# CompVis/zigma

Measured on AMD Instinct MI355X. Metric: denoiser-forward latents/sec (BxL tokens/s), ZigMa d=640 L=32^2, higher is better.
Workload: dtype bf16; 1 GPU; readme_text_b64: ZigMa(in_ch=3,img=32,E=640,depth=18,zigzagN8,has_text 77x768), B=64/GPU, bf16, one forward per step; global_batch=64, seq_len=1024, parallelism=batch-sharded x1

## Files before the change

include/zigma_hip.h:

```cpp
#ifndef ZIGMA_HIP_H_
#define ZIGMA_HIP_H_

#include <stdint.h>

#ifdef __cplusplus
extern "C" {
#endif

#define ZIGMA_ABI_VERSION 10

#define ZIGMA_SCAN_Z_PREACTIVATED 2
#define ZIGMA_SCAN_ACCUMULATE 4
#define ZIGMA_SCAN_PROBE_V1 0x100
#define ZIGMA_SCAN_PROBE_PRIO_SHIFT 9
#define ZIGMA_SCAN_PROBE_R5_SHIFT 10

#define ZIGMA_SCAN_KERNEL_GENERIC 1
#define ZIGMA_SCAN_KERNEL_TOK 2
#define ZIGMA_SCAN_KERNEL_TOK2 3

typedef enum zigma_status {
    ZIGMA_OK = 0,
    ZIGMA_ERR_NULL = -1,
    ZIGMA_ERR_SHAPE = -2,
// ... 202 lines not shown

int zigma_scale_reduce_bwd(const zigma_glue_bwd_params_t *p, void *stream);

typedef struct zigma_xattn_params {
    int32_t batch, seqlen, n_ctx, heads, head_dim;
    int32_t dtype;
    int32_t flags;
    float scale;
    int64_t q_batch_stride, q_row_stride;
    int64_t k_batch_stride, k_row_stride;
    int64_t v_batch_stride, v_row_stride;
    int64_t o_batch_stride, o_row_stride;
    const void *q, *k, *v;
    void *out;
} zigma_xattn_params_t;

int zigma_cross_attn_fwd(const zigma_xattn_params_t *p, void *stream);

typedef struct zigma_xattn_bwd_params {
    int32_t batch, seqlen, n_ctx, heads, head_dim;
    int32_t dtype;
    int32_t flags;
    float scale;
    int32_t chunks;
    int32_t pad_;
    int64_t q_batch_stride, q_row_stride;
    int64_t k_batch_stride, k_row_stride;
    int64_t v_batch_stride, v_row_stride;
    int64_t do_batch_stride, do_row_stride;
    int64_t dq_batch_stride, dq_row_stride;
    const void *q, *k, *v, *dout;
    void *dq, *dk_part, *dv_part;
} zigma_xattn_bwd_params_t;

int zigma_cross_attn_bwd_chunks(int seqlen);
int zigma_cross_attn_bwd(const zigma_xattn_bwd_params_t *p, void *stream);

typedef struct zigma_xproj_params {
    int64_t m;
    int32_t n, k;
    int32_t dtype;
    int32_t flags;
    int64_t x_row_stride, w_row_stride, out_row_stride;
    const void *x, *w;
    void *out;
} zigma_xproj_params_t;

int zigma_x_proj_fwd(const zigma_xproj_params_t *p, void *stream);

typedef struct zigma_conv_xproj_params {
    int32_t batch, seqlen, dim, n;
    int32_t dtype;
    int32_t flags;
    int64_t x_batch_stride, x_l_stride;
    int64_t u_batch_stride, u_l_stride;
    int64_t w_row_stride, out_row_stride;
    const void *x, *conv_weight, *conv_bias, *w;
    void *u, *out;
    const int32_t *x_row_index;
} zigma_conv_xproj_params_t;

int zigma_conv_x_proj_fwd(const zigma_conv_xproj_params_t *p, void *stream);

#define ZIGMA_LINEAR_WS 0x4000
#define ZIGMA_LINEAR_SM 0x8000
typedef struct zigma_linear_params {
    int64_t m;
    int32_t n, k;
    int32_t dtype;
    int32_t flags;
    int32_t silu_from_col;
    int32_t pad_;
    int64_t x_row_stride, w_row_stride, out_row_stride;
    const void *x, *w;
    const void *bias;
    void *out;
    const void *residual, *gate;
    int64_t res_row_stride, gate_batch_stride;
    int32_t rows_per_batch, pad2_;
} zigma_linear_params_t;

int zigma_linear_fwd(const zigma_linear_params_t *p, void *stream);

typedef struct zigma_linear_wgrad_params {
    int64_t m;
    int32_t n, k;
    int32_t dtype;
    int32_t out_dtype;
    int32_t slabs;
    int32_t flags;
    int64_t dy_row_stride, x_row_stride, out_row_stride;
    const void *dy, *x;
    void *out;
    void *workspace;
    int64_t workspace_bytes;
} zigma_linear_wgrad_params_t;

int64_t zigma_linear_wgrad_workspace_bytes(const zigma_linear_wgrad_params_t *p);
int zigma_linear_wgrad(const zigma_linear_wgrad_params_t *p, void *stream);

typedef struct zigma_linear_split_params {
    int64_t m;
    int32_t n, k;
    int32_t passes;
    int32_t flags;
    int64_t x_row_stride, w_hi_row_stride, w_lo_row_stride, out_row_stride;
    const void *x;
    const void *w_hi, *w_lo;
    const void *bias;
    void *out;
} zigma_linear_split_params_t;

int zigma_linear_f32_split(const zigma_linear_split_params_t *p, void *stream);

typedef struct zigma_patch_embed_params {
    int32_t batch, in_chans, height, width, patch, embed_dim;
    int32_t dtype;
    int32_t flags;
    int64_t x_batch_stride, x_chan_stride, x_row_stride;
    int64_t pos_row_stride, out_batch_stride, out_row_stride;
    const void *x, *weight, *bias, *pos;
    void *out;
} zigma_patch_embed_params_t;

typedef struct zigma_timestep_embed_params {
    int32_t batch, dim;
    int32_t dtype;
    int32_t flags;
    int64_t out_row_stride;
    const void *t, *freqs;
    void *out;
} zigma_timestep_embed_params_t;

typedef struct zigma_final_layer_params {
    int64_t rows;
    int32_t cols, n_out;
    int32_t dtype;
    int32_t flags;
    float eps;
    int32_t pad_;
    int64_t x_row_stride, out_row_stride;
    const void *x, *weight, *bias;
    void *out;
} zigma_final_layer_params_t;

typedef struct zigma_skinny_params {
    int32_t m, n, k;
    int32_t dtype;
    int32_t flags;
    int32_t pad_;
    int64_t x_row_stride, w_row_stride, out_row_stride;
    const void *x, *w, *bias;
    void *out;
} zigma_skinny_params_t;

int zigma_patch_embed_fwd(const zigma_patch_embed_params_t *p, void *stream);
int zigma_timestep_embed_fwd(const zigma_timestep_embed_params_t *p, void *stream);
int zigma_final_layer_fwd(const zigma_final_layer_params_t *p, void *stream);
int zigma_skinny_linear_fwd(const zigma_skinny_params_t *p, void *stream);

typedef struct zigma_calib_params {
    int32_t mode, iters;
    int64_t bytes;
    const void *src;
    void *dst;
} zigma_calib_params_t;
// ... 11 lines not shown
```

zigma_amd/_lib.py:

```python
import ctypes as C
import os

import torch

_HERE = os.path.dirname(os.path.abspath(__file__))
LIB_PATH = os.environ.get("ZIGMA_AMD_LIB") or os.path.join(_HERE, "lib", "libzigma_hip.so")

F32, F16, BF16 = 0, 1, 2
_DT = {torch.float32: F32, torch.float16: F16, torch.bfloat16: BF16}

i32, i64, vp, f32 = C.c_int32, C.c_int64, C.c_void_p, C.c_float


class ScanParams(C.Structure):
    _fields_ = (
        [(n, i32) for n in ("batch", "dim", "seqlen", "dstate", "n_groups", "is_variable_B", "is_variable_C",
                            "delta_softplus", "io_dtype", "bc_dtype", "chunk_len", "flags")]
        + [(n, i64) for n in (
            "u_batch_stride", "u_d_stride", "u_l_stride",
            "delta_batch_stride", "delta_d_stride", "delta_l_stride",
            "z_batch_stride", "z_d_stride", "z_l_stride",
            "out_batch_stride", "out_d_stride", "out_l_stride",
            "out_z_batch_stride", "out_z_d_stride", "out_z_l_stride",
            "A_d_stride", "A_dstate_stride",
# ... 65 lines not shown
    _fields_ = ([(n, i32) for n in ("rows", "cols", "is_rms", "x_dtype", "res_dtype", "w_dtype")]
                + [("eps", f32), ("flags", i32)]
                + [(n, i64) for n in ("xsum_row_stride", "dy_row_stride", "dres_out_row_stride", "dx_row_stride",
                                      "dres_row_stride")]
                + [(n, vp) for n in ("xsum", "weight", "dy", "dresidual_out", "dx", "dresidual", "dweight", "dbias",
                                     "workspace")]
                + [("workspace_bytes", i64)])


class XAttnParams(C.Structure):
    _fields_ = ([(n, i32) for n in ("batch", "seqlen", "n_ctx", "heads", "head_dim", "dtype", "flags")] + [("scale", f32)]
                + [(n, i64) for n in ("q_batch_stride", "q_row_stride", "k_batch_stride", "k_row_stride", "v_batch_stride",
                                      "v_row_stride", "o_batch_stride", "o_row_stride")]
                + [(n, vp) for n in ("q", "k", "v", "out")])


class XAttnBwdParams(C.Structure):
    _fields_ = ([(n, i32) for n in ("batch", "seqlen", "n_ctx", "heads", "head_dim", "dtype", "flags")] + [("scale", f32)]
                + [("chunks", i32), ("pad_", i32)]
                + [(n, i64) for n in ("q_batch_stride", "q_row_stride", "k_batch_stride", "k_row_stride", "v_batch_stride",
                                      "v_row_stride", "do_batch_stride", "do_row_stride", "dq_batch_stride", "dq_row_stride")]
                + [(n, vp) for n in ("q", "k", "v", "dout", "dq", "dk_part", "dv_part")])


class PatchEmbedParams(C.Structure):
    _fields_ = ([(n, i32) for n in ("batch", "in_chans", "height", "width", "patch", "embed_dim", "dtype", "flags")]
                + [(n, i64) for n in ("x_batch_stride", "x_chan_stride", "x_row_stride", "pos_row_stride", "out_batch_stride", "out_row_stride")]
                + [(n, vp) for n in ("x", "weight", "bias", "pos", "out")])


class TimestepEmbedParams(C.Structure):
    _fields_ = [("batch", i32), ("dim", i32), ("dtype", i32), ("flags", i32), ("out_row_stride", i64), ("t", vp), ("freqs", vp), ("out", vp)]


class FinalLayerParams(C.Structure):
    _fields_ = ([("rows", i64), ("cols", i32), ("n_out", i32), ("dtype", i32), ("flags", i32), ("eps", f32), ("pad_", i32),
                 ("x_row_stride", i64), ("out_row_stride", i64)] + [(n, vp) for n in ("x", "weight", "bias", "out")])


class SkinnyParams(C.Structure):
    _fields_ = ([(n, i32) for n in ("m", "n", "k", "dtype", "flags", "pad_")] + [(n, i64) for n in ("x_row_stride", "w_row_stride", "out_row_stride")]
                + [(n, vp) for n in ("x", "w", "bias", "out")])


class GlueBwdParams(C.Structure):
    _fields_ = ([("rows", i64), ("cols", i32), ("rows_per_batch", i32), ("dtype", i32), ("flags", i32), ("s_add", f32), ("pad_", i32)]
                + [(n, i64) for n in ("dy_row_stride", "a_row_stride", "out_row_stride", "s_batch_stride")]
                + [(n, vp) for n in ("dy", "a", "s", "out", "r1", "r2")])


class CalibParams(C.Structure):
    _fields_ = [("mode", i32), ("iters", i32), ("bytes", i64), ("src", vp), ("dst", vp)]


class XProjParams(C.Structure):
    _fields_ = ([("m", i64), ("n", i32), ("k", i32), ("dtype", i32), ("flags", i32)]
                + [(n, i64) for n in ("x_row_stride", "w_row_stride", "out_row_stride")] + [(n, vp) for n in ("x", "w", "out")])


class ConvXProjParams(C.Structure):
    _fields_ = ([(n, i32) for n in ("batch", "seqlen", "dim", "n", "dtype", "flags")]
                + [(n, i64) for n in ("x_batch_stride", "x_l_stride", "u_batch_stride", "u_l_stride", "w_row_stride", "out_row_stride")]
                + [(n, vp) for n in ("x", "conv_weight", "conv_bias", "w", "u", "out", "x_row_index")])


class LinearParams(C.Structure):
    _fields_ = ([("m", i64), ("n", i32), ("k", i32), ("dtype", i32), ("flags", i32), ("silu_from_col", i32), ("pad_", i32)]
                + [(n, i64) for n in ("x_row_stride", "w_row_stride", "out_row_stride")] + [(n, vp) for n in ("x", "w", "bias", "out")]
                + [("residual", vp), ("gate", vp), ("res_row_stride", i64), ("gate_batch_stride", i64), ("rows_per_batch", i32), ("pad2_", i32)])


class LinearWgradParams(C.Structure):
    _fields_ = ([("m", i64), ("n", i32), ("k", i32), ("dtype", i32), ("out_dtype", i32), ("slabs", i32), ("flags", i32)]
                + [(n, i64) for n in ("dy_row_stride", "x_row_stride", "out_row_stride")] + [(n, vp) for n in ("dy", "x", "out", "workspace")]
                + [("workspace_bytes", i64)])


class LinearSplitParams(C.Structure):
    _fields_ = ([("m", i64), ("n", i32), ("k", i32), ("passes", i32), ("flags", i32)]
                + [(n, i64) for n in ("x_row_stride", "w_hi_row_stride", "w_lo_row_stride", "out_row_stride")]
                + [(n, vp) for n in ("x", "w_hi", "w_lo", "bias", "out")])


EXPORTS = ("zigma_linear_fwd", "zigma_linear_f32_split", "zigma_linear_wgrad","zigma_linear_wgrad_workspace_bytes", "zigma_conv_x_proj_fwd", "zigma_scale_reduce_bwd", "zigma_selective_scan_fwd", "zigma_causal_conv1d_fwd", "zigma_add_norm_fwd", "zigma_dt_proj_softplus_fwd", "zigma_cross_attn_fwd", "zigma_x_proj_fwd", "zigma_selective_scan_bwd",
           "zigma_selective_scan_bwd_workspace_bytes", "zigma_causal_conv1d_bwd",
           "zigma_causal_conv1d_bwd_workspace_bytes", "zigma_add_norm_bwd", "zigma_add_norm_bwd_workspace_bytes",
           "zigma_strerror",
           "zigma_cross_attn_bwd", "zigma_cross_attn_bwd_chunks", "zigma_patch_embed_fwd", "zigma_timestep_embed_fwd", "zigma_final_layer_fwd",
           "zigma_skinny_linear_fwd", "zigma_calib_launch", "zigma_abi_version", "zigma_last_kernel")

_lib = None


def lib():
    global _lib
    if _lib is None:
        if not os.path.exists(LIB_PATH):
            raise RuntimeError(
                f"zigma_amd: {LIB_PATH} not built — run `python -m zigma_amd.build` (hipcc, gfx950). "
                "There is no CPU or eager fallback for the HIP ops.")
        L = C.CDLL(LIB_PATH)
        for name, st in (("zigma_selective_scan_fwd", ScanParams), ("zigma_causal_conv1d_fwd", ConvParams),
                         ("zigma_add_norm_fwd", NormParams), ("zigma_dt_proj_softplus_fwd", DtProjParams),
                         ("zigma_selective_scan_bwd", ScanBwdParams), ("zigma_causal_conv1d_bwd", ConvBwdParams),
                         ("zigma_add_norm_bwd", NormBwdParams), ("zigma_cross_attn_fwd", XAttnParams), ("zigma_cross_attn_bwd", XAttnBwdParams), ("zigma_patch_embed_fwd", PatchEmbedParams),
                         ("zigma_timestep_embed_fwd", TimestepEmbedParams), ("zigma_final_layer_fwd", FinalLayerParams), ("zigma_skinny_linear_fwd", SkinnyParams), ("zigma_x_proj_fwd", XProjParams),
                         ("zigma_linear_fwd", LinearParams), ("zigma_conv_x_proj_fwd", ConvXProjParams), ("zigma_scale_reduce_bwd", GlueBwdParams), ("zigma_calib_launch", CalibParams),
                         ("zigma_linear_wgrad", LinearWgradParams), ("zigma_linear_f32_split", LinearSplitParams)):
            fn = getattr(L, name)
            fn.argtypes = [C.POINTER(st), vp]
            fn.restype = C.c_int
        for name, st in (("zigma_selective_scan_bwd_workspace_bytes", ScanBwdParams),
                         ("zigma_causal_conv1d_bwd_workspace_bytes", ConvBwdParams),
                         ("zigma_add_norm_bwd_workspace_bytes", NormBwdParams),
                         ("zigma_linear_wgrad_workspace_bytes", LinearWgradParams)):
            fn = getattr(L, name)
            fn.argtypes = [C.POINTER(st)]
            fn.restype = C.c_int64
        L.zigma_cross_attn_bwd_chunks.argtypes = [C.c_int]
        L.zigma_cross_attn_bwd_chunks.restype = C.c_int
        L.zigma_strerror.argtypes = [C.c_int]
        L.zigma_strerror.restype = C.c_char_p
        L.zigma_abi_version.restype = C.c_int
        L.zigma_last_kernel.restype = C.c_char_p
        if L.zigma_abi_version() != 10:
            raise RuntimeError("zigma_amd: libzigma_hip.so ABI version mismatch")
        _lib = L
    return _lib


def last_kernel():
    return lib().zigma_last_kernel().decode()


def dtype_id(t):
    try:
        return _DT[t.dtype]
    except KeyError:
        raise RuntimeError(f"zigma_amd: unsupported dtype {t.dtype}")


def ptr(t):
    return None if t is None else t.data_ptr()


def require_device(*tensors):
    dev = None
    for t in tensors:
        if t is None:
            continue
        if not t.is_cuda:
            raise RuntimeError("zigma_amd: HIP kernels need tensors on a GPU device (no CPU fallback); got a "
                               f"{t.device} tensor")
        if dev is None:
            dev = t.device
        elif t.device != dev:
            raise RuntimeError("zigma_amd: all tensors must be on the same device")
    return dev


def workspace(fn_name, params, device):
    nbytes = getattr(lib(), fn_name + "_workspace_bytes")(C.byref(params))
    ws = torch.empty(max(int(nbytes), 16), device=device, dtype=torch.uint8)
    params.workspace, params.workspace_bytes = ws.data_ptr(), nbytes
    return ws


TRACE = None


def call(fn_name, params, device):
    L = lib()
    with torch.cuda.device(device):
        stream = torch.cuda.current_stream(device).cuda_stream
        rc = getattr(L, fn_name)(C.byref(params), C.c_void_p(stream))
    if rc != 0:
        raise RuntimeError(f"{fn_name}: {L.zigma_strerror(rc).decode()} (status {rc})")
    if TRACE is not None:
        TRACE.append((fn_name, L.zigma_last_kernel().decode(), params))
```

zigma_amd/build.py:

```python
import hashlib
import os
import subprocess
import sys
from concurrent.futures import ThreadPoolExecutor

HERE = os.path.dirname(os.path.abspath(__file__))
ROOT = os.path.dirname(HERE)
CSRC = os.path.join(HERE, "csrc")
OBJ = os.path.join(HERE, "build")
LIB = os.path.join(HERE, "lib", "libzigma_hip.so")
SOURCES = ["api.hip", "selective_scan.hip", "scan_tok_bf16.hip", "scan_tok_f16.hip", "scan_tok_f32.hip",
           "causal_conv1d.hip", "add_norm.hip", "dt_proj.hip", "scan_bwd.hip", "conv_bwd.hip", "norm_bwd.hip", "cross_attn.hip", "cross_attn_bwd.hip", "x_proj.hip", "linear.hip", "linear4w.hip", "linear_ws.hip", "linear_sm.hip", "conv_x_proj.hip", "glue_bwd.hip", "embed.hip", "skinny_linear.hip", "calib.hip", "wgrad.hip", "linear_split.hip"]
HIPCC = os.environ.get("HIPCC", "/opt/rocm/bin/hipcc")
FLAGS = ["--offload-arch=gfx950", "-O3", "-std=c++17", "-fPIC", "-ffp-contract=fast", "-fno-slp-vectorize",
         "-I" + os.path.join(ROOT, "include"), "-I" + CSRC]


_VGPR_MFMA = ["-mllvm", "-amdgpu-mfma-vgpr-form=1"]
_RES = ["-Rpass-analysis=kernel-resource-usage"]
SOURCE_FLAGS = {"cross_attn.hip": _VGPR_MFMA, "scan_tok_bf16.hip": _RES, "scan_tok_f16.hip": _RES, "wgrad.hip": _RES, "linear_split.hip": _RES}
NO_SCRATCH_KERNELS = ("scan_tok2_kernel", "wgrad_kernel", "wgrad_reduce_kernel", "linear_split_kernel")


def check_no_scratch(remarks, src):
    import re
    bad, seen, name = [], 0, None
    for ln in remarks.splitlines():
        m = re.search(r"remark: Function Name: (\S+)", ln)
        if m:
            name = m.group(1) if any(k in m.group(1) for k in NO_SCRATCH_KERNELS) else None
            seen += name is not None
            continue
        m = re.search(r"remark:\s+(ScratchSize \[bytes/lane\]|SGPRs Spill|VGPRs Spill): (\d+)", ln)
        if m and name and int(m.group(2)) != 0:
            bad.append((name, m.group(1), int(m.group(2))))
    if bad or not seen:
        raise RuntimeError(f"{src}: {' / '.join(NO_SCRATCH_KERNELS)} must not spill or use scratch (scan_tok2_kernel: inline-asm d16_hi row loads are invisible to the register allocator): "
                           f"{bad if bad else 'no instantiation found in the remarks'}")
    return seen


GENERATED_F16_INC = os.path.join(CSRC, "linear4w_body_f16.inc")


def ensure_generated(verbose=True):
    import importlib.util
    spec = importlib.util.spec_from_file_location("zigma_linear4w_gen", os.path.join(CSRC, "gen", "linear4w_gen.py"))
    gen = importlib.util.module_from_spec(spec)
    spec.loader.exec_module(gen)
    tmp = GENERATED_F16_INC + ".tmp"
    gen.emit_inc_f16(tmp)
    if os.path.exists(GENERATED_F16_INC) and open(GENERATED_F16_INC).read() == open(tmp).read():
        os.remove(tmp)
        return GENERATED_F16_INC
    os.replace(tmp, GENERATED_F16_INC)
    if verbose:
        print(f"generated {GENERATED_F16_INC}", flush=True)
    return GENERATED_F16_INC


def _digest(paths, extra=()):
    h = hashlib.sha256()
    for pth in sorted(paths):
        h.update(os.path.basename(pth).encode())
        h.update(open(pth, "rb").read())
    for e in extra:
        h.update(str(e).encode())
    return h.hexdigest()


def build(force=False, verbose=True, sources=None, lib=None, extra_flags=()):
    sources = sources or SOURCES
    lib = lib or LIB
    obj_dir = OBJ if lib == LIB else OBJ + "_" + os.path.splitext(os.path.basename(lib))[0]
    os.makedirs(obj_dir, exist_ok=True)
    os.makedirs(os.path.dirname(lib), exist_ok=True)
    ensure_generated(verbose)
    headers = [os.path.join(CSRC, f) for f in os.listdir(CSRC) if f.endswith((".h", ".inc"))]
    headers.append(os.path.join(ROOT, "include", "zigma_hip.h"))
    stamp = lib + ".srchash"
    want = _digest([os.path.join(CSRC, s) for s in sources] + headers, extra=list(FLAGS) + list(extra_flags) + [str(sorted(SOURCE_FLAGS.items()))])
    if not force and os.path.exists(lib) and os.path.exists(stamp) and open(stamp).read().strip() == want:
        if verbose:
            print(f"{lib} is up to date (source hash {want[:12]})")
        return lib

    def run(cmd):
        if verbose:
            print(" ".join(cmd), flush=True)
        subprocess.run(cmd, check=True)

    objs, jobs = [], []
    for src in sources:
        s_path = os.path.join(CSRC, src)
        o_path = os.path.join(obj_dir, src.replace(".hip", ".o"))
        o_stamp = o_path + ".srchash"
        src_flags = SOURCE_FLAGS.get(src, [])
        o_want = _digest([s_path] + headers, extra=list(FLAGS) + list(extra_flags) + src_flags)
        objs.append(o_path)
        if force or not os.path.exists(o_path) or not os.path.exists(o_stamp) or open(o_stamp).read().strip() != o_want:
            jobs.append(([HIPCC, *FLAGS, *extra_flags, *src_flags, "-c", s_path, "-o", o_path], o_stamp, o_want))

    def compile_one(job):
        cmd, o_stamp, o_want = job
# ... 21 lines not shown
```

zigma_amd/model_zigma.py:

```python
import math
import os
from functools import partial
from typing import Optional

import numpy as np
import torch
import torch.nn as nn
import torch.nn.functional as F
import torch.utils.checkpoint
from torch import Tensor

from .attention import attention_math, cross_attn, cross_attn_bwd_eligible, cross_attn_eligible, cross_attn_train
from . import embed as _embed
from .layernorm import RMSNorm, block_norm, glue_bwd_eligible, layer_norm_fn, rms_norm_fn, scale_reduce_bwd
from .linear import plan, project, run
from .mamba_simple import Mamba
from .scan_paths import hilbert_path, reverse_permut_np, zigzag_path


def modulate(x, shift, scale):
    return x * (1 + scale.unsqueeze(1)) + shift.unsqueeze(1)


class _ModulateFn(torch.autograd.Function):

    @staticmethod
    def forward(ctx, x, shift, scale):
        ctx.save_for_backward(x, scale)
        return torch.addcmul(shift.unsqueeze(1), x, (1 + scale).unsqueeze(1))

    @staticmethod
    def backward(ctx, dy):
        x, scale = ctx.saved_tensors
        if glue_bwd_eligible(dy, x, scale):
            dx, dscale, dshift = scale_reduce_bwd(dy, x, scale, s_add=1.0, want_sum=True)
            return dx, dshift, dscale
        dx = dy * (1 + scale).unsqueeze(1)
        return dx, dy.sum(1), (dy * x).sum(1)


class _GatedAddFn(torch.autograd.Function):

    @staticmethod
    def forward(ctx, base, gate, branch):
        ctx.save_for_backward(gate, branch)
        return torch.addcmul(base, gate.unsqueeze(1), branch)

    @staticmethod
    def backward(ctx, dy):
        gate, branch = ctx.saved_tensors
        if glue_bwd_eligible(dy, branch, gate):
            dbranch, dgate, _ = scale_reduce_bwd(dy, branch, gate)
            return dy, dgate, dbranch
        return dy, (dy * branch).sum(1), dy * gate.unsqueeze(1)


class PatchEmbed(nn.Module):

    def __init__(self, img_size=224, patch_size=16, in_chans=3, embed_dim=768, bias=True):
        super().__init__()
        self.img_size = (img_size, img_size)
        self.patch_size = (patch_size, patch_size)
        self.grid_size = (img_size // patch_size, img_size // patch_size)
        self.num_patches = self.grid_size[0] * self.grid_size[1]
        self.proj = nn.Conv2d(in_chans, embed_dim, kernel_size=patch_size, stride=patch_size, bias=bias)

    def forward(self, x, pos=None):
        Bsz, Cin, H, W = x.shape
        p = self.patch_size[0]
        no_grad = not (torch.is_grad_enabled() and (x.requires_grad or self.proj.weight.requires_grad
                                                    or (self.proj.bias is not None and self.proj.bias.requires_grad) or (pos is not None and pos.requires_grad)))
        if no_grad and _embed.patch_embed_eligible(x, self.proj.weight, self.proj.bias, pos):
            return _embed.patch_embed(x, self.proj.weight, self.proj.bias, pos)
        cols = x.reshape(Bsz, Cin, H // p, p, W // p, p).permute(0, 2, 4, 1, 3, 5).reshape(Bsz, -1, Cin * p * p)
        tok = F.linear(cols, self.proj.weight.reshape(self.proj.weight.shape[0], -1), self.proj.bias)
        return tok if pos is None else tok + pos


class PatchEmbed_Video(PatchEmbed):
    def forward(self, x, pos=None):
        Bsz, T = x.shape[:2]
        tok = super().forward(x.reshape((Bsz * T,) + x.shape[2:]))
        tok = tok.reshape(Bsz, -1, tok.shape[-1])
        return tok if pos is None else tok + pos


class CrossAttention(nn.Module):
    def __init__(self, query_dim, context_dim=None, heads=8, dim_head=64, dropout=0.0):
        super().__init__()
        inner_dim = dim_head * heads
        context_dim = query_dim if context_dim is None else context_dim
        self.scale = dim_head ** -0.5
        self.heads = heads
        self.to_q = nn.Linear(query_dim, inner_dim, bias=False)
        self.to_k = nn.Linear(context_dim, inner_dim, bias=False)
        self.to_v = nn.Linear(context_dim, inner_dim, bias=False)
        self.to_out = nn.Sequential(nn.Linear(inner_dim, query_dim), nn.Dropout(dropout))

    def _proj_out(self, o, residual, gate):
        lin = self.to_out[0]
        if residual is None or self.training:
            y = self.to_out[1](project("to_out", o, lin.weight, lin.bias))
            return y if residual is None else torch.addcmul(residual, gate.unsqueeze(1), y)
        return project("to_out", o, lin.weight, lin.bias, residual=residual, gate=gate)

    def forward(self, x, text, mask=None, kv=None, residual=None, gate=None):
        Bsz, L, _ = x.shape
        H = self.heads
        k, v = kv[:2] if kv is not None else (self.to_k(text), self.to_v(text))
        q = project("to_q", x, self.to_q.weight, self.to_q.bias)
        needs_grad = torch.is_grad_enabled() and (q.requires_grad or k.requires_grad or v.requires_grad)
        if cross_attn_eligible(q, k, v, H) and (not needs_grad or cross_attn_bwd_eligible(q, k, v, H)):
            if needs_grad:
                return self._proj_out(cross_attn_train(q, k, v, H, self.scale), residual, gate)
            return self._proj_out(cross_attn(q, k, v, H, self.scale), residual, gate)
        return self._proj_out(attention_math(q, k.reshape(Bsz, k.shape[1], -1), v.reshape(Bsz, v.shape[1], -1), H, self.scale), residual, gate)


def drop_path(x, drop_prob: float = 0.0, training: bool = False, scale_by_keep: bool = True):
    if drop_prob == 0.0 or not training:
        return x
    keep = 1 - drop_prob
    mask = x.new_empty((x.shape[0],) + (1,) * (x.ndim - 1)).bernoulli_(keep)
    if keep > 0.0 and scale_by_keep:
        mask.div_(keep)
    return x * mask


class DropPath(nn.Module):
    def __init__(self, drop_prob: float = 0.0, scale_by_keep: bool = True):
        super().__init__()
        self.drop_prob = drop_prob
        self.scale_by_keep = scale_by_keep

    def forward(self, x):
        return drop_path(x, self.drop_prob, self.training, self.scale_by_keep)


class TimestepEmbedder(nn.Module):

    def __init__(self, hidden_size, dtype, frequency_embedding_size=256):
        super().__init__()
        self.mlp = nn.Sequential(nn.Linear(frequency_embedding_size, hidden_size, bias=True), nn.SiLU(),
                                 nn.Linear(hidden_size, hidden_size, bias=True))
        self.dtype = dtype
        self.frequency_embedding_size = frequency_embedding_size
        self.register_buffer("_freqs", self.frequencies(frequency_embedding_size, dtype), persistent=False)

    @staticmethod
    def frequencies(dim, dtype, max_period=10000):
        half = dim // 2
        return torch.exp(-math.log(max_period) * torch.arange(start=0, end=half, dtype=dtype) / half)

    @staticmethod
    def timestep_embedding(t, dim, dtype, max_period=10000, freqs=None):
        if freqs is None:
            freqs = TimestepEmbedder.frequencies(dim, dtype, max_period).to(device=t.device)
        args = t[:, None].float() * freqs[None]
        embedding = torch.cat([torch.cos(args), torch.sin(args)], dim=-1)
        if dim % 2:
            embedding = torch.cat([embedding, torch.zeros_like(embedding[:, :1])], dim=-1)
        return embedding

    def forward(self, t):
        freqs = self._freqs if self._freqs.dtype == self.dtype else self._freqs.to(self.dtype)
        l1, l2 = self.mlp[0], self.mlp[2]
        if self.frequency_embedding_size % 2 == 0 and _embed.timestep_embed_eligible(t, freqs):
            t_freq = _embed.timestep_embed(t, freqs, self.frequency_embedding_size)
        else:
            t_freq = self.timestep_embedding(t, self.frequency_embedding_size, dtype=self.dtype, freqs=freqs).to(dtype=self.dtype)
        if _embed.skinny_linear_eligible(t_freq, l1.weight, l1.bias):
            h = _embed.skinny_linear(t_freq, l1.weight, l1.bias)
            if _embed.skinny_linear_eligible(h, l2.weight, l2.bias):
                return _embed.skinny_linear(h, l2.weight, l2.bias, silu=True)
            return l2(F.silu(h))
        return self.mlp(t_freq)


class LabelEmbedder(nn.Module):
    def __init__(self, num_classes, hidden_size, dropout_prob):
        super().__init__()
        use_cfg_embedding = dropout_prob > 0
        self.embedding_table = nn.Embedding(num_classes + use_cfg_embedding, hidden_size)
        self.num_classes = num_classes
        self.dropout_prob = dropout_prob

    def token_drop(self, labels, force_drop_ids=None):
        if force_drop_ids is None:
            drop_ids = torch.rand(labels.shape[0], device=labels.device) < self.dropout_prob
        else:
            drop_ids = force_drop_ids == 1
        return torch.where(drop_ids, self.num_classes, labels)

    def forward(self, labels, train, force_drop_ids=None):
        if (train and self.dropout_prob > 0) or (force_drop_ids is not None):
            labels = self.token_drop(labels, force_drop_ids)
        return self.embedding_table(labels)


class FinalLayer(nn.Module):
    def __init__(self, hidden_size, patch_size, out_channels, cond=False):
        super().__init__()
        self.norm_final = nn.LayerNorm(hidden_size, elementwise_affine=False, eps=1e-6)
        self.linear = nn.Linear(hidden_size, patch_size * patch_size * out_channels, bias=True)
        if cond:
            self.adaLN_modulation = nn.Sequential(nn.SiLU(), nn.Linear(hidden_size, 2 * hidden_size, bias=True))

    def forward(self, x, c=None):
        if c is None and _embed.final_layer_eligible(x, self.linear.weight, self.linear.bias):
            return _embed.final_layer(x, self.linear.weight, self.linear.bias, self.norm_final.eps)
        x = layer_norm_fn(x, None, None, eps=self.norm_final.eps)
        if c is not None:
            shift, scale = self.adaLN_modulation(c).chunk(2, dim=1)
            x = modulate(x, shift, scale)
        return self.linear(x)


class Pending:
    __slots__ = ("base", "branch", "gate")

    def __init__(self, base, branch=None, gate=None):
        self.base, self.branch, self.gate = base, branch, gate

    def materialize(self):
        if self.branch is None:
            return self.base
        return torch.addcmul(self.base, self.gate.unsqueeze(1), self.branch)


def _text_linear(x, weight, bias=None):
    k = x.shape[-1]
    m = x.numel() // k
    xp = x.new_zeros(-(-m // 256) * 256, k)
    xp[:m] = x.reshape(m, k)
    r = plan("text", xp, weight, bias)
    if r.kernel == "library":
        return F.linear(x, weight, bias)
    return run(r, xp, weight, bias)[:m].view(*x.shape[:-1], weight.shape[0])


FUSE_OUT_PROJ_ADD = True
FUSE_OUT_PROJ_ADD_NO_TEXT = True
from . import _knobs
_knobs.apply(globals(), "model_zigma")


class Block(nn.Module):
    def __init__(self, dim, mixer_cls, has_text=False, norm_cls=nn.LayerNorm, fused_add_norm=False,
                 residual_in_fp32=False, drop_path=0.0, skip=False):
        super().__init__()
        self.residual_in_fp32 = residual_in_fp32
        self.fused_add_norm = fused_add_norm
        self.has_text = has_text
        self.mixer = mixer_cls(dim)
        self.norm = norm_cls(dim)
        self.drop_path = DropPath(drop_path) if drop_path > 0.0 else nn.Identity()
        if self.fused_add_norm:
            assert isinstance(self.norm, (nn.LayerNorm, RMSNorm)), "Only LayerNorm and RMSNorm are supported for fused_add_norm"
        self.skip_linear = nn.Linear(2 * dim, dim) if skip else None
        adaln_num = 3 * 2 if self.has_text else 3
        self.adaLN_modulation = nn.Sequential(nn.SiLU(), nn.Linear(dim, adaln_num * dim, bias=True))
        if self.has_text:
            self.msa = CrossAttention(query_dim=dim, context_dim=dim, heads=8, dim_head=64, dropout=0.0)
            self.norm_msa = nn.LayerNorm(dim, elementwise_affine=False, eps=1e-6)

    def forward_fused(self, pend: Pending, residual, c, text=None, mod=None, kv=None):
        E = pend.base.shape[-1]
        if mod is None:
            mod = self.adaLN_modulation(c)
        is_rms = isinstance(self.norm, RMSNorm)
        _, residual, n, xm = block_norm(pend.base, self.norm.weight, self.norm.bias, residual, self.norm.eps, is_rms,
                                        residual_in_fp32=self.residual_in_fp32, branch=pend.branch, gate=pend.gate,
                                        shift=mod[:, 0:E], scale=mod[:, E:2 * E])
        g = mod[:, 2 * E:3 * E]
        fuse = FUSE_OUT_PROJ_ADD if self.has_text else FUSE_OUT_PROJ_ADD_NO_TEXT
        y, fused = self.mixer.forward_gated(xm, n, g) if fuse else (self.mixer(xm), False)
        pend = Pending(y) if fused else Pending(n, y, g)
        if not self.has_text:
            return pend, residual
        h, _, _, xa = block_norm(pend.base, None, None, None, self.norm_msa.eps, False, residual_in_fp32=False, branch=pend.branch,
                                 gate=pend.gate, shift=mod[:, 3 * E:4 * E], scale=mod[:, 4 * E:5 * E], want_x=True, want_y=False, want_res_out=False)
        h = pend.base if fused else h
        return Pending(self.msa(xa, text=text, mask=None, kv=kv, residual=h, gate=mod[:, 5 * E:6 * E])), residual

    def forward(self, x: Tensor, residual: Optional[Tensor] = None, c=None, text=None, inference_params=None, skip=None):
        if self.skip_linear is not None:
            x = self.skip_linear(torch.cat([x, skip], dim=-1))
        if not self.fused_add_norm:
            residual = x if residual is None else residual + self.drop_path(x)
            n = self.norm(residual.to(dtype=self.norm.weight.dtype))
            if self.residual_in_fp32:
                residual = residual.to(torch.float32)
            mod = self.adaLN_modulation(c).chunk(6 if self.has_text else 3, dim=1)
            h = n + mod[2].unsqueeze(1) * self.mixer(modulate(n, mod[0], mod[1]))
            if self.has_text:
                xa = modulate(layer_norm_fn(h, None, None, eps=self.norm_msa.eps), mod[3], mod[4])
                h = h + mod[5].unsqueeze(1) * self.msa(xa, text=text, mask=None)
            return h, residual
        if torch.is_grad_enabled() and (x.requires_grad or any(q.requires_grad for q in self.parameters())):
            return self.forward_train(x, residual, c, text)
        if residual is not None:
            x = self.drop_path(x)
        pend, residual = self.forward_fused(Pending(x), residual, c, text)
        return pend.materialize(), residual

    def forward_train(self, x, residual, c, text=None):
        fn = rms_norm_fn if isinstance(self.norm, RMSNorm) else layer_norm_fn
        x, residual = fn(x if residual is None else self.drop_path(x), self.norm.weight, self.norm.bias, residual=residual,
                         prenorm=True, residual_in_fp32=self.residual_in_fp32, eps=self.norm.eps)
        mod = self.adaLN_modulation(c).chunk(6 if self.has_text else 3, dim=1)
        x = _GatedAddFn.apply(x, mod[2], self.mixer(_ModulateFn.apply(x, mod[0], mod[1])))
        if self.has_text:
            xa = _ModulateFn.apply(layer_norm_fn(x, None, None, eps=self.norm_msa.eps), mod[3], mod[4])
            x = _GatedAddFn.apply(x, mod[5], self.msa(xa, text=text, mask=None))
        return x, residual


def create_block(d_model, ssm_cfg=None, has_text=False, norm_epsilon=1e-5, drop_path=0.0, rms_norm=False,
                 residual_in_fp32=False, fused_add_norm=False, skip=False, layer_idx=None, device=None, dtype=None,
                 scan_type="none", **block_kwargs):
    if ssm_cfg is None:
        ssm_cfg = {}
    factory_kwargs = {"device": device, "dtype": dtype}
    mixer_cls = partial(Mamba, layer_idx=layer_idx, scan_type=scan_type, **ssm_cfg, **block_kwargs, **factory_kwargs)
    norm_cls = partial(nn.LayerNorm if not rms_norm else RMSNorm, eps=norm_epsilon, **factory_kwargs)
    block = Block(d_model, mixer_cls, has_text=has_text, norm_cls=norm_cls, drop_path=drop_path,
                  fused_add_norm=fused_add_norm, residual_in_fp32=residual_in_fp32, skip=skip)
    block.layer_idx = layer_idx
    return block


def _init_weights(module, n_layer, initializer_range=0.02, rescale_prenorm_residual=True, n_residuals_per_layer=1):
    if isinstance(module, nn.Linear):
        if module.bias is not None and not getattr(module.bias, "_no_reinit", False):
            nn.init.zeros_(module.bias)
    elif isinstance(module, nn.Embedding):
        nn.init.normal_(module.weight, std=initializer_range)
    if rescale_prenorm_residual:
        for name, p in module.named_parameters():
            if name in ["out_proj.weight", "fc2.weight"]:
                nn.init.kaiming_uniform_(p, a=math.sqrt(5))
                with torch.no_grad():
                    p /= math.sqrt(n_residuals_per_layer * n_layer)


def get_1d_sincos_pos_embed_from_grid(embed_dim, pos):
    assert embed_dim % 2 == 0
    omega = 1.0 / 10000 ** (np.arange(embed_dim // 2, dtype=np.float64) / (embed_dim / 2.0))
    out = np.outer(pos.reshape(-1), omega)
    return np.concatenate([np.sin(out), np.cos(out)], axis=1)


def get_2d_sincos_pos_embed(embed_dim, grid_size, cls_token=False, extra_tokens=0):
    coords = np.arange(grid_size, dtype=np.float32)
    gw, gh = np.meshgrid(coords, coords)
    emb = np.concatenate([get_1d_sincos_pos_embed_from_grid(embed_dim // 2, gw),
                          get_1d_sincos_pos_embed_from_grid(embed_dim // 2, gh)], axis=1)
    if cls_token and extra_tokens > 0:
        emb = np.concatenate([np.zeros([extra_tokens, embed_dim]), emb], axis=0)
    return emb


# ... 235 lines not shown
```

Baseline: 3.772 million tokens/s.

## Fuse cross-attention LayerNorm and adaLN modulate into the to_q GEMM

Adds a new HIP kernel that computes LayerNorm and the shift/scale modulation on each 32-token tile, keeping the normalized rows in registers and feeding them straight into MFMA matmuls against the to_q weight (N=512). The goal is to stop materializing the modulated activation for cross-attention, saving a global write and read and a separate norm kernel launch per text block. It applies only in bias-free, no-grad, fused-pending cases above a token threshold, and falls back to the old path otherwise. The kernel is hand-scheduled (LDS staging, manual waitcnts) for fixed N and K, so it risks lower GEMM efficiency than the tuned library or routed kernel.

New measurement: 3.912 million tokens/s (median of 6 runs). +3.7%, better.

```diff
diff --git a/include/zigma_hip.h b/include/zigma_hip.h
--- a/include/zigma_hip.h
+++ b/include/zigma_hip.h
@@ -308,6 +308,20 @@
 
 int zigma_linear_fwd(const zigma_linear_params_t *p, void *stream);
 
+typedef struct zigma_norm_linear_params {
+    int64_t m;
+    int32_t n, k;
+    int32_t dtype;
+    int32_t flags;
+    int32_t rows_per_batch;
+    float eps;
+    int64_t x_row_stride, w_row_stride, out_row_stride, mod_batch_stride;
+    const void *x, *w, *shift, *scale;
+    void *out;
+} zigma_norm_linear_params_t;
+
+int zigma_norm_linear_fwd(const zigma_norm_linear_params_t *p, void *stream);
+
 typedef struct zigma_linear_wgrad_params {
     int64_t m;
     int32_t n, k;
diff --git a/zigma_amd/_lib.py b/zigma_amd/_lib.py
--- a/zigma_amd/_lib.py
+++ b/zigma_amd/_lib.py
@@ -171,7 +171,13 @@
                 + [(n, vp) for n in ("x", "w_hi", "w_lo", "bias", "out")])
 
 
-EXPORTS = ("zigma_linear_fwd", "zigma_linear_f32_split", "zigma_linear_wgrad","zigma_linear_wgrad_workspace_bytes", "zigma_conv_x_proj_fwd", "zigma_scale_reduce_bwd", "zigma_selective_scan_fwd", "zigma_causal_conv1d_fwd", "zigma_add_norm_fwd", "zigma_dt_proj_softplus_fwd", "zigma_cross_attn_fwd", "zigma_x_proj_fwd", "zigma_selective_scan_bwd",
+class NormLinearParams(C.Structure):
+    _fields_ = ([("m", i64), ("n", i32), ("k", i32), ("dtype", i32), ("flags", i32), ("rows_per_batch", i32), ("eps", f32)]
+                + [(n, i64) for n in ("x_row_stride", "w_row_stride", "out_row_stride", "mod_batch_stride")]
+                + [(n, vp) for n in ("x", "w", "shift", "scale", "out")])
+
+
+EXPORTS = ("zigma_linear_fwd", "zigma_norm_linear_fwd", "zigma_linear_f32_split", "zigma_linear_wgrad","zigma_linear_wgrad_workspace_bytes", "zigma_conv_x_proj_fwd", "zigma_scale_reduce_bwd", "zigma_selective_scan_fwd", "zigma_causal_conv1d_fwd", "zigma_add_norm_fwd", "zigma_dt_proj_softplus_fwd", "zigma_cross_attn_fwd", "zigma_x_proj_fwd", "zigma_selective_scan_bwd",
            "zigma_selective_scan_bwd_workspace_bytes", "zigma_causal_conv1d_bwd",
            "zigma_causal_conv1d_bwd_workspace_bytes", "zigma_add_norm_bwd", "zigma_add_norm_bwd_workspace_bytes",
            "zigma_strerror",
@@ -195,7 +201,7 @@
                          ("zigma_add_norm_bwd", NormBwdParams), ("zigma_cross_attn_fwd", XAttnParams), ("zigma_cross_attn_bwd", XAttnBwdParams), ("zigma_patch_embed_fwd", PatchEmbedParams),
                          ("zigma_timestep_embed_fwd", TimestepEmbedParams), ("zigma_final_layer_fwd", FinalLayerParams), ("zigma_skinny_linear_fwd", SkinnyParams), ("zigma_x_proj_fwd", XProjParams),
                          ("zigma_linear_fwd", LinearParams), ("zigma_conv_x_proj_fwd", ConvXProjParams), ("zigma_scale_reduce_bwd", GlueBwdParams), ("zigma_calib_launch", CalibParams),
-                         ("zigma_linear_wgrad", LinearWgradParams), ("zigma_linear_f32_split", LinearSplitParams)):
+                         ("zigma_linear_wgrad", LinearWgradParams), ("zigma_linear_f32_split", LinearSplitParams), ("zigma_norm_linear_fwd", NormLinearParams)):
             fn = getattr(L, name)
             fn.argtypes = [C.POINTER(st), vp]
             fn.restype = C.c_int
diff --git a/zigma_amd/build.py b/zigma_amd/build.py
--- a/zigma_amd/build.py
+++ b/zigma_amd/build.py
@@ -10,7 +10,7 @@
 OBJ = os.path.join(HERE, "build")
 LIB = os.path.join(HERE, "lib", "libzigma_hip.so")
 SOURCES = ["api.hip", "selective_scan.hip", "scan_tok_bf16.hip", "scan_tok_f16.hip", "scan_tok_f32.hip",
-           "causal_conv1d.hip", "add_norm.hip", "dt_proj.hip", "scan_bwd.hip", "conv_bwd.hip", "norm_bwd.hip", "cross_attn.hip", "cross_attn_bwd.hip", "x_proj.hip", "linear.hip", "linear4w.hip", "linear_ws.hip", "linear_sm.hip", "conv_x_proj.hip", "glue_bwd.hip", "embed.hip", "skinny_linear.hip", "calib.hip", "wgrad.hip", "linear_split.hip"]
+           "causal_conv1d.hip", "add_norm.hip", "dt_proj.hip", "scan_bwd.hip", "conv_bwd.hip", "norm_bwd.hip", "cross_attn.hip", "cross_attn_bwd.hip", "x_proj.hip", "linear.hip", "linear4w.hip", "linear_ws.hip", "linear_sm.hip", "conv_x_proj.hip", "glue_bwd.hip", "embed.hip", "skinny_linear.hip", "calib.hip", "wgrad.hip", "linear_split.hip", "norm_linear.hip"]
 HIPCC = os.environ.get("HIPCC", "/opt/rocm/bin/hipcc")
 FLAGS = ["--offload-arch=gfx950", "-O3", "-std=c++17", "-fPIC", "-ffp-contract=fast", "-fno-slp-vectorize",
          "-I" + os.path.join(ROOT, "include"), "-I" + CSRC]
@@ -18,8 +18,8 @@
 
 _VGPR_MFMA = ["-mllvm", "-amdgpu-mfma-vgpr-form=1"]
 _RES = ["-Rpass-analysis=kernel-resource-usage"]
-SOURCE_FLAGS = {"cross_attn.hip": _VGPR_MFMA, "scan_tok_bf16.hip": _RES, "scan_tok_f16.hip": _RES, "wgrad.hip": _RES, "linear_split.hip": _RES}
-NO_SCRATCH_KERNELS = ("scan_tok2_kernel", "wgrad_kernel", "wgrad_reduce_kernel", "linear_split_kernel")
+SOURCE_FLAGS = {"cross_attn.hip": _VGPR_MFMA, "scan_tok_bf16.hip": _RES, "scan_tok_f16.hip": _RES, "wgrad.hip": _RES, "linear_split.hip": _RES, "norm_linear.hip": _RES}
+NO_SCRATCH_KERNELS = ("scan_tok2_kernel", "wgrad_kernel", "wgrad_reduce_kernel", "linear_split_kernel", "norm_linear_kernel")
 
 
 def check_no_scratch(remarks, src):
diff --git a/zigma_amd/csrc/norm_linear.hip b/zigma_amd/csrc/norm_linear.hip
--- /dev/null
+++ b/zigma_amd/csrc/norm_linear.hip
@@ -0,0 +1,204 @@
+#include "norm_linear_plan.h"
+#include "zigma_common.h"
+
+namespace zigma {
+namespace nl {
+
+typedef float f32x16 __attribute__((ext_vector_type(16)));
+typedef unsigned u32x4 __attribute__((ext_vector_type(4)));
+typedef unsigned u32x2 __attribute__((ext_vector_type(2)));
+typedef __attribute__((address_space(3))) unsigned char *lds_ptr_t;
+typedef const __attribute__((address_space(1))) void *gbl_ptr_t;
+
+template <int OFF> __device__ __forceinline__ void lds_rd(u32x4 &d, unsigned addr) {
+    asm volatile("ds_read_b128 %0, %1 offset:%2" : "=v"(d) : "v"(addr), "i"(OFF));
+}
+template <int N> __device__ __forceinline__ void settle2(u32x4 &a, u32x4 &b) {
+    static_assert(N == 0 || N == 2 || N == 4, "");
+    if (N == 0) asm volatile("s_waitcnt lgkmcnt(0)" : "+v"(a), "+v"(b));
+    else if (N == 2) asm volatile("s_waitcnt lgkmcnt(2)" : "+v"(a), "+v"(b));
+    else asm volatile("s_waitcnt lgkmcnt(4)" : "+v"(a), "+v"(b));
+}
+__device__ __forceinline__ void settle4(u32x4 &a, u32x4 &b, u32x4 &c, u32x4 &d) {
+    asm volatile("s_waitcnt lgkmcnt(0)" : "+v"(a), "+v"(b), "+v"(c), "+v"(d));
+}
+__device__ __forceinline__ void wait_vm(int n) {
+    if (n >= 8) asm volatile("s_waitcnt vmcnt(8)" ::: "memory");
+    else if (n >= 4) asm volatile("s_waitcnt vmcnt(4)" ::: "memory");
+    else asm volatile("s_waitcnt vmcnt(0)" ::: "memory");
+}
+template <typename T> __device__ __forceinline__ v2f unpk(unsigned w) { return v2f{lo16<T>(w), hi16<T>(w)}; }
+
+template <int KS, typename T>
+__global__ __launch_bounds__(64 * kNlWaves, KS <= 10 ? 2 : 1) void norm_linear_kernel(const zigma_norm_linear_params_t p) {
+    constexpr int NF = KS * 4;
+    constexpr int NXS = KS;
+    constexpr int WPP = KS / 2;
+    constexpr int NPASS = kNlN / kNlPass;
+    constexpr int NST = kNlStages, SB = kNlStageBytes;
+    constexpr int kTileOff = NST * SB, kTileBytes = kNlTok * kNlOutPitch;
+    static_assert(KS % 2 == 0 && WPP >= NST && NXS >= NST && NST == 3 && SB == 16384 && kNlPass == 64 && kNlWaves == 4 && kNlTok == 32, "");
+    __shared__ __attribute__((aligned(1024))) unsigned char smem[kTileOff + kNlWaves * kTileBytes];
+    const int tid = threadIdx.x, lane = tid & 63;
+    const int wave = __builtin_amdgcn_readfirstlane(tid >> 6);
+    const int j = lane & 31, kh = lane >> 5, l3 = lane >> 3;
+    const int64_t m0 = (static_cast<int64_t>(blockIdx.x) * kNlWaves + wave) * kNlTok;
+    const unsigned smem_lds = static_cast<unsigned>(reinterpret_cast<uintptr_t>((lds_ptr_t)(smem)));
+
+    const int64_t x_pitch = p.x_row_stride * 2, w_pitch = p.w_row_stride * 2, o_pitch = p.out_row_stride * 2;
+    const unsigned char *xb = reinterpret_cast<const unsigned char *>(p.x) + m0 * x_pitch;
+    const unsigned char *wb = reinterpret_cast<const unsigned char *>(p.w) + static_cast<int64_t>(wave) * 8 * w_pitch;
+    const unsigned slot = static_cast<unsigned>((lane & 7) ^ (l3 >> 1));
+    const unsigned xoff0 = static_cast<unsigned>(l3 * x_pitch) + (slot << 4), xoff1 = static_cast<unsigned>(l3 * x_pitch) + ((slot ^ 4u) << 4);
+    const unsigned woff = static_cast<unsigned>(l3 * w_pitch) + ((slot ^ static_cast<unsigned>((wave & 1) << 2)) << 4);
+
+    auto issue_x = [&](int st, int bi) {
+        unsigned char *dst = smem + bi * SB + wave * 4096;
+        const unsigned char *src = xb + st * 128;
+#pragma unroll
+        for (int i = 0; i < 4; ++i)
+            __builtin_amdgcn_global_load_lds((gbl_ptr_t)(src + static_cast<int64_t>(i) * 8 * x_pitch + ((i & 1) ? xoff1 : xoff0)), (lds_ptr_t)(dst) + i * 1024, 16, 0, 0);
+    };
+    auto issue_w = [&](int pass, int kk, int bi) {
+        unsigned char *dst = smem + bi * SB + wave * 1024;
+        const unsigned char *src = wb + static_cast<int64_t>(pass) * kNlPass * w_pitch + kk * 256 + woff;
+#pragma unroll
+        for (int i = 0; i < 4; ++i) {
+            const int c = i >> 1, h = i & 1;
+            __builtin_amdgcn_global_load_lds((gbl_ptr_t)(src + static_cast<int64_t>(h) * 32 * w_pitch + c * 128), (lds_ptr_t)(dst) + c * 8192 + h * 4096, 16, 0, 0);
+        }
+    };
+
+    const unsigned lrd = smem_lds + static_cast<unsigned>(j * 128 + ((kh ^ ((j >> 1) & 7)) << 4));
+
+    u32x4 xf[NF];
+    v2f sum2 = {0.f, 0.f};
+    issue_x(0, 0);
+    issue_x(1, 1);
+#pragma unroll
+    for (int s = 0; s < NXS; ++s) {
+        wait_vm(4);
+        __builtin_amdgcn_s_barrier();
+        if (s + 2 < NXS) issue_x(s + 2, (s + 2) % NST);
+        else issue_w(0, s + 2 - NXS, (s + 2) % NST);
+        const unsigned a = lrd + (s % NST) * SB + wave * 4096;
+#pragma unroll
+        for (int ks = 0; ks < 4; ++ks) lds_rd<0>(xf[s * 4 + ks], a ^ (ks << 5));
+        settle4(xf[s * 4], xf[s * 4 + 1], xf[s * 4 + 2], xf[s * 4 + 3]);
+#pragma unroll
+        for (int ks = 0; ks < 4; ++ks)
+#pragma unroll
+            for (int d = 0; d < 4; ++d) sum2 += unpk<T>(xf[s * 4 + ks][d]);
+    }
+
+    {
+        float sum = sum2.x + sum2.y;
+        sum += __shfl_xor(sum, 32, 64);
+        const float mean = sum / p.k;
+        v2f var2 = {0.f, 0.f};
+#pragma unroll
+        for (int f = 0; f < NF; ++f) {
+            asm volatile("" : "+v"(xf[f]));
+#pragma unroll
+            for (int d = 0; d < 4; ++d) {
+                const v2f dl = unpk<T>(xf[f][d]) - mean;
+                var2 += dl * dl;
+            }
+        }
+        float var = var2.x + var2.y;
+        var += __shfl_xor(var, 32, 64);
+        const float rstd = rsqrtf(var / p.k + p.eps);
+        const int64_t b = (m0 + j) / p.rows_per_batch;
+        const unsigned char *shp = reinterpret_cast<const unsigned char *>(p.shift) + b * p.mod_batch_stride * 2 + kh * 16;
+        const unsigned char *scp = reinterpret_cast<const unsigned char *>(p.scale) + b * p.mod_batch_stride * 2 + kh * 16;
+#pragma unroll
+        for (int f = 0; f < NF; ++f) {
+            const u32x4 sh = *reinterpret_cast<const u32x4 *>(shp + f * 32), sc = *reinterpret_cast<const u32x4 *>(scp + f * 32);
+            asm volatile("" : "+v"(xf[f]));
+#pragma unroll
+            for (int d = 0; d < 4; ++d) {
+                const v2f y = (unpk<T>(xf[f][d]) - mean) * rstd;
+                const v2f yr = unpk<T>(pack2_pk<T>(y.x, y.y));
+                const v2f o = yr * (1.f + unpk<T>(sc[d])) + unpk<T>(sh[d]);
+                xf[f][d] = pack2_pk<T>(o.x, o.y);
+            }
+            if (f % 4 == 3) asm volatile("" ::: "memory");
+        }
+    }
+
+    const unsigned tile = smem_lds + kTileOff + wave * kTileBytes;
+    unsigned char *ob = reinterpret_cast<unsigned char *>(p.out) + (m0 + l3) * o_pitch + (lane & 7) * 16;
+    int buf = NXS % NST;
+#pragma unroll 1
+    for (int pass = 0; pass < NPASS; ++pass) {
+        f32x16 acc[2];
+        acc[0] = f32x16{};
+        acc[1] = f32x16{};
+#pragma unroll
+        for (int kk = 0; kk < WPP; ++kk) {
+            {
+                const int younger = (pass == NPASS - 1 && kk == WPP - 1) ? 0 : 4;
+                const int stores = (pass > 0 && kk < NST - 1) ? 4 : 0;
+                wait_vm(younger + stores);
+            }
+            __builtin_amdgcn_s_barrier();
+            {
+                const int prev = buf == 0 ? NST - 1 : buf - 1;
+                if (kk + 2 < WPP) issue_w(pass, kk + 2, prev);
+                else if (pass + 1 < NPASS) issue_w(pass + 1, kk + 2 - WPP, prev);
+            }
+            const unsigned a0 = lrd + buf * SB;
+            u32x4 wf[3][2];
+            auto reads = [&](int g) {
+                const unsigned a = a0 ^ ((g & 3) << 5);
+                if (g < 4) { lds_rd<0>(wf[g % 3][0], a); lds_rd<4096>(wf[g % 3][1], a); }
+                else { lds_rd<8192>(wf[g % 3][0], a); lds_rd<8192 + 4096>(wf[g % 3][1], a); }
+            };
+            reads(0);
+            reads(1);
+#pragma unroll
+            for (int g = 0; g < 8; ++g) {
+                if (g + 2 < 8) { reads(g + 2); settle2<4>(wf[g % 3][0], wf[g % 3][1]); }
+                else if (g + 1 < 8) settle2<2>(wf[g % 3][0], wf[g % 3][1]);
+                else settle2<0>(wf[g % 3][0], wf[g % 3][1]);
+                const frag8_t<T> xa = __builtin_bit_cast(frag8_t<T>, xf[kk * 8 + g]);
+                acc[0] = mfma_32x32x16<T>(__builtin_bit_cast(frag8_t<T>, wf[g % 3][0]), xa, acc[0]);
+                acc[1] = mfma_32x32x16<T>(__builtin_bit_cast(frag8_t<T>, wf[g % 3][1]), xa, acc[1]);
+            }
+            buf = buf + 1 == NST ? 0 : buf + 1;
+        }
+#pragma unroll
+        for (int nb = 0; nb < 2; ++nb)
+#pragma unroll
+            for (int q = 0; q < 4; ++q) {
+                const u32x2 pk = {pack2_pk<T>(acc[nb][q * 4], acc[nb][q * 4 + 1]), pack2_pk<T>(acc[nb][q * 4 + 2], acc[nb][q * 4 + 3])};
+                asm volatile("ds_write_b64 %0, %1" ::"v"(tile + j * kNlOutPitch + nb * 64 + q * 16 + kh * 8), "v"(pk) : "memory");
+            }
+        u32x4 t[4];
+#pragma unroll
+        for (int i = 0; i < 4; ++i) lds_rd<0>(t[i], tile + (i * 8 + l3) * kNlOutPitch + (lane & 7) * 16);
+        settle4(t[0], t[1], t[2], t[3]);
+#pragma unroll
+        for (int i = 0; i < 4; ++i) *reinterpret_cast<u32x4 *>(ob + static_cast<int64_t>(i) * 8 * o_pitch + pass * (2 * kNlPass)) = t[i];
+    }
+}
+
+}
+}
+
+using namespace zigma;
+
+extern "C" int zigma_norm_linear_fwd(const zigma_norm_linear_params_t *pp, void *stream_) {
+    if (!pp) return ZIGMA_ERR_NULL;
+    (void)hipGetLastError();
+    const zigma_norm_linear_params_t &p = *pp;
+    const NormLinearPlan plan = plan_norm_linear(p);
+    if (!plan.kernel) return plan.status;
+    hipStream_t stream = static_cast<hipStream_t>(stream_);
+    const dim3 grid(plan.grid), block(plan.block);
+#define ZIGMA_NL(KS_) ZIGMA_DISPATCH_16BIT(p.dtype, T, hipLaunchKernelGGL((nl::norm_linear_kernel<KS_, T>), grid, block, 0, stream, p))
+    if (plan.ksteps == 8) { ZIGMA_NL(8) } else if (plan.ksteps == 10) { ZIGMA_NL(10) } else { ZIGMA_NL(12) }
+#undef ZIGMA_NL
+    set_last_kernel(plan.kernel);
+    return check_launch();
+}
diff --git a/zigma_amd/csrc/norm_linear_plan.h b/zigma_amd/csrc/norm_linear_plan.h
--- /dev/null
+++ b/zigma_amd/csrc/norm_linear_plan.h
@@ -0,0 +1,46 @@
+#pragma once
+#include <stdint.h>
+
+#include "zigma_hip.h"
+
+namespace zigma {
+
+constexpr int kNlWaves = 4, kNlTok = 32;
+constexpr int kNlTile = kNlWaves * kNlTok;
+constexpr int kNlN = 512;
+constexpr int kNlPass = 64;
+constexpr int kNlStageBytes = 16384, kNlStages = 3;
+constexpr int kNlOutPitch = 2 * kNlPass + 16;
+
+struct NormLinearPlan {
+    int status = ZIGMA_OK;
+    const char *kernel = nullptr;
+    unsigned grid = 0, block = 0;
+    int ksteps = 0;
+};
+
+inline bool nl_al(const void *q, uintptr_t bytes) { return reinterpret_cast<uintptr_t>(q) % bytes == 0; }
+
+inline NormLinearPlan plan_norm_linear(const zigma_norm_linear_params_t &p) {
+    NormLinearPlan s;
+    auto refuse = [&s](int status) { s.status = status; return s; };
+    if (p.m < 0 || p.n < 1 || p.k < 1 || p.rows_per_batch < 1) return refuse(ZIGMA_ERR_SHAPE);
+    if (p.flags != 0) return refuse(ZIGMA_ERR_UNSUPPORTED);
+    if (p.m == 0) return s;
+    if (!p.x || !p.w || !p.shift || !p.scale || !p.out) return refuse(ZIGMA_ERR_NULL);
+    if (p.dtype != ZIGMA_BF16 && p.dtype != ZIGMA_F16) return refuse(ZIGMA_ERR_DTYPE);
+    if (p.n != kNlN || (p.k != 512 && p.k != 640 && p.k != 768)) return refuse(ZIGMA_ERR_SHAPE);
+    if (p.m % kNlTile != 0 || p.m / kNlTile > 0x7fffffff) return refuse(ZIGMA_ERR_SHAPE);
+    if (p.m % p.rows_per_batch != 0) return refuse(ZIGMA_ERR_SHAPE);
+    if (p.x_row_stride < p.k || p.w_row_stride < p.k || p.out_row_stride < p.n || p.mod_batch_stride < 0) return refuse(ZIGMA_ERR_SHAPE);
+    if (p.x_row_stride * 16 > 0x7fffffff || p.w_row_stride * 16 > 0x7fffffff) return refuse(ZIGMA_ERR_SHAPE);
+    if (p.x_row_stride % 8 != 0 || p.w_row_stride % 8 != 0 || p.out_row_stride % 8 != 0 || p.mod_batch_stride % 8 != 0 || !nl_al(p.x, 16) || !nl_al(p.w, 16) ||
+        !nl_al(p.shift, 16) || !nl_al(p.scale, 16) || !nl_al(p.out, 16))
+        return refuse(ZIGMA_ERR_STRIDE);
+    s.ksteps = p.k / 64;
+    s.grid = static_cast<unsigned>(p.m / kNlTile); s.block = 64 * kNlWaves;
+    s.kernel = p.k == 512 ? "norm_linear_k512" : p.k == 640 ? "norm_linear_k640" : "norm_linear_k768";
+    return s;
+}
+
+}
diff --git a/zigma_amd/model_zigma.py b/zigma_amd/model_zigma.py
--- a/zigma_amd/model_zigma.py
+++ b/zigma_amd/model_zigma.py
@@ -14,6 +14,8 @@
 from . import embed as _embed
 from .layernorm import RMSNorm, block_norm, glue_bwd_eligible, layer_norm_fn, rms_norm_fn, scale_reduce_bwd
 from .linear import plan, project, run
+from .norm_linear import norm_linear, norm_linear_eligible
+from . import routing
 from .mamba_simple import Mamba
 from .scan_paths import hilbert_path, reverse_permut_np, zigzag_path
 
@@ -104,11 +106,12 @@
             return y if residual is None else torch.addcmul(residual, gate.unsqueeze(1), y)
         return project("to_out", o, lin.weight, lin.bias, residual=residual, gate=gate)
 
-    def forward(self, x, text, mask=None, kv=None, residual=None, gate=None):
-        Bsz, L, _ = x.shape
+    def forward(self, x, text, mask=None, kv=None, residual=None, gate=None, q=None):
+        Bsz, L, _ = x.shape if q is None else q.shape
         H = self.heads
         k, v = kv[:2] if kv is not None else (self.to_k(text), self.to_v(text))
-        q = project("to_q", x, self.to_q.weight, self.to_q.bias)
+        if q is None:
+            q = project("to_q", x, self.to_q.weight, self.to_q.bias)
         needs_grad = torch.is_grad_enabled() and (q.requires_grad or k.requires_grad or v.requires_grad)
         if cross_attn_eligible(q, k, v, H) and (not needs_grad or cross_attn_bwd_eligible(q, k, v, H)):
             if needs_grad:
@@ -241,8 +244,23 @@
 
 FUSE_OUT_PROJ_ADD = True
 FUSE_OUT_PROJ_ADD_NO_TEXT = True
+FUSE_NORM_TO_Q = True
+NORM_TO_Q_MIN_TOKENS = 65536
 from . import _knobs
 _knobs.apply(globals(), "model_zigma")
+
+
+def fuse_norm_to_q(pend, to_q, shift, scale):
+    if not FUSE_NORM_TO_Q or pend.branch is not None:
+        return False
+    x = pend.base
+    if x.dim() != 3:
+        return False
+    tokens = x.shape[0] * x.shape[1]
+    n, k = to_q.weight.shape
+    if tokens < NORM_TO_Q_MIN_TOKENS or routing.route("to_q", tokens, n, k).kernel == "library":
+        return False
+    return norm_linear_eligible(x, to_q.weight, shift, scale, to_q.bias)
 
 
 class Block(nn.Module):
@@ -278,6 +296,9 @@
         pend = Pending(y) if fused else Pending(n, y, g)
         if not self.has_text:
             return pend, residual
+        if fuse_norm_to_q(pend, self.msa.to_q, mod[:, 3 * E:4 * E], mod[:, 4 * E:5 * E]):
+            q = norm_linear(pend.base, self.msa.to_q.weight, mod[:, 3 * E:4 * E], mod[:, 4 * E:5 * E], self.norm_msa.eps)
+            return Pending(self.msa(None, text=text, mask=None, kv=kv, residual=pend.base, gate=mod[:, 5 * E:6 * E], q=q)), residual
         h, _, _, xa = block_norm(pend.base, None, None, None, self.norm_msa.eps, False, residual_in_fp32=False, branch=pend.branch,
                                  gate=pend.gate, shift=mod[:, 3 * E:4 * E], scale=mod[:, 4 * E:5 * E], want_x=True, want_y=False, want_res_out=False)
         h = pend.base if fused else h
diff --git a/zigma_amd/norm_linear.py b/zigma_amd/norm_linear.py
--- /dev/null
+++ b/zigma_amd/norm_linear.py
@@ -0,0 +1,45 @@
+import torch
+
+from . import _lib
+
+TILE = 128
+N_OUT = 512
+K_SERVED = (512, 640, 768)
+MFMA_DTYPES = (torch.bfloat16, torch.float16)
+
+
+def norm_linear_shape_ok(m, n, k, rows_per_batch):
+    return n == N_OUT and k in K_SERVED and m > 0 and m % TILE == 0 and m // TILE <= 0x7fffffff and rows_per_batch >= 1 and m % rows_per_batch == 0
+
+
+def norm_linear_eligible(x, weight, shift, scale, bias=None):
+    if bias is not None or x.dim() != 3 or weight.dim() != 2 or shift.dim() != 2 or scale.dim() != 2:
+        return False
+    if not (x.is_cuda and x.dtype in MFMA_DTYPES and weight.dtype == x.dtype and shift.dtype == x.dtype and scale.dtype == x.dtype):
+        return False
+    if torch.is_grad_enabled() and (x.requires_grad or weight.requires_grad or shift.requires_grad or scale.requires_grad):
+        return False
+    Bsz, L, k = x.shape
+    n = weight.shape[0]
+    if weight.shape[1] != k or shift.shape != (Bsz, k) or scale.shape != (Bsz, k) or not norm_linear_shape_ok(Bsz * L, n, k, L):
+        return False
+    if x.stride(2) != 1 or weight.stride(1) != 1 or shift.stride(1) != 1 or scale.stride(1) != 1 or x.stride(0) != L * x.stride(1):
+        return False
+    if shift.stride(0) != scale.stride(0) or shift.stride(0) < 0 or not (k <= x.stride(1) < 1 << 27) or not (k <= weight.stride(0) < 1 << 27):
+        return False
+    return all(s % 8 == 0 for s in (x.stride(1), weight.stride(0), shift.stride(0))) and all(t.data_ptr() % 16 == 0 for t in (x, weight, shift, scale))
+
+
+def norm_linear(x, weight, shift, scale, eps, out=None):
+    dev = _lib.require_device(x, weight, shift, scale, out)
+    Bsz, L, k = x.shape
+    n = weight.shape[0]
+    if out is None:
+        out = torch.empty(Bsz * L, n, device=x.device, dtype=x.dtype)
+    o2 = out if out.dim() == 2 else out.view(-1, n)
+    P = _lib.NormLinearParams()
+    P.m, P.n, P.k, P.dtype, P.flags, P.rows_per_batch, P.eps = Bsz * L, n, k, _lib.dtype_id(x), 0, L, float(eps)
+    P.x_row_stride, P.w_row_stride, P.out_row_stride, P.mod_batch_stride = x.stride(1), weight.stride(0), o2.stride(0), shift.stride(0)
+    P.x, P.w, P.shift, P.scale, P.out = _lib.ptr(x), _lib.ptr(weight), _lib.ptr(shift), _lib.ptr(scale), _lib.ptr(o2)
+    _lib.call("zigma_norm_linear_fwd", P, dev)
+    return out.view(Bsz, L, n) if out.dim() == 2 and out.is_contiguous() else out
```
